# MarkJhonBao/InfantPoseEstimation_GaussianBias

Hardware: AMD Instinct MI355X
Metric: images/sec (train fwd+bwd) HRFormer-S 256x192 (higher is better)
Workload: dtype bf16; 1 GPU; HRFormer-small + fusion head, 256x192 -> 64x48, K=17, train step fwd+bwd+AdamW, DropPath 0.1, BN train; global_batch=64, per_gpu_batch=64, parallelism=dp1, launch=hipGraph replay, branches on concurrent HIP streams

## Files before the change

### infantposeestimation_gaussianbias_amd/csrc/pk_bn_out1x1.hip

```cpp
#include <stdlib.h>

#include "pk_rowops.h"

#define BO_ROWS 128
#define BO_GRID 512
#define BO_MIN_ROWS 32768
#define BO_SMALL_ROWS 32768

struct BnOutArgs {
    const uint4* raw;
    const uint16_t* w;
    const uint16_t* g;
    const uint8_t* mask_in;
    uint8_t* mask_out;
    const float* v0;
    const float* v1;
    const float* gamma;
    const float* sums;
    const float* bias;
    float* out;
    uint4* t_out;
    uint4* draw;
    float* part;
    float inv_count;
    int small;
    int64_t rows;
    int N, N8, hw, softplus;
    int nb, rpb;
};

template <int C>
struct BoGeom {
    static constexpr int CPR = C / 8;
    static constexpr int RPI = 64 / CPR;
    static constexpr int NLD = 16 / RPI;
    static constexpr int TP = C + 8;
    static constexpr int RL = 256 / CPR;
    static constexpr int TILE_BYTES = (16 * TP * 2 > RL * C * 4) ? 16 * TP * 2 : RL * C * 4;
};

__device__ __forceinline__ void bo_wave_sync() {
    __builtin_amdgcn_fence(__ATOMIC_ACQ_REL, "wavefront");
    __builtin_amdgcn_wave_barrier();
}

template <int C, int NB>
__global__ void __launch_bounds__(256, 2) k_bn_out1x1_fwd(BnOutArgs p) {
    using G = BoGeom<C>;
    constexpr int CPR = G::CPR, RPI = G::RPI, NLD = G::NLD, TP = G::TP;
    extern __shared__ __attribute__((aligned(16))) unsigned char bo_smem[];
    uint16_t* sW = reinterpret_cast<uint16_t*>(bo_smem);
    const int tid = threadIdx.x, lane = tid & 63, wave = tid >> 6;
    uint16_t* tile = reinterpret_cast<uint16_t*>(bo_smem + NB * 16 * TP * 2) + wave * 16 * TP;
    const int frow = lane & 15, fkc = lane >> 4;
    const int lch = lane % CPR, lrw = lane / CPR;
    const int64_t rows = p.rows;
    const int ntiles = (int)((rows + BO_ROWS - 1) / BO_ROWS);
    auto block_base = [&](int it) -> int64_t {
        const int64_t t = (int64_t)blockIdx.x + (int64_t)(it >> 1) * gridDim.x;
        return t < ntiles ? t * BO_ROWS + wave * 32 + (it & 1) * 16 : -1;
    };
    auto load_raw = [&](uint4 (&rv)[NLD], int64_t base) {
#pragma unroll
        for (int i = 0; i < NLD; ++i) {
            const int64_t row = base + i * RPI + lrw;
            rv[i] = make_uint4(0u, 0u, 0u, 0u);
            if (base >= 0 && row < rows) rv[i] = p.raw[(size_t)row * CPR + lch];
        }
    };
    uint4 rv[NLD], rn[NLD];
    int64_t base = block_base(0);
// ... 43 lines not shown
#pragma unroll
        for (int a = 0; a < NB; ++a) acc[a] = (f32x4){0.f, 0.f, 0.f, 0.f};
#pragma unroll
        for (int ks = 0; ks < C / 32; ++ks) {
            const bf16x8 tf = *reinterpret_cast<const bf16x8*>(&tile[frow * TP + (ks * 4 + fkc) * 8]);
#pragma unroll
            for (int a = 0; a < NB; ++a) {
                const bf16x8 wf = *reinterpret_cast<const bf16x8*>(&sW[(a * 16 + frow) * TP + (ks * 4 + fkc) * 8]);
                acc[a] = __builtin_amdgcn_mfma_f32_16x16x32_bf16(wf, tf, acc[a], 0, 0, 0);
            }
        }
        const int64_t row = base + frow;
        if (row < rows) {
            const int bb = (int)(row / p.hw), pix = (int)(row - (int64_t)bb * p.hw);
            float* o = p.out + (size_t)bb * p.N * p.hw + pix;
#pragma unroll
            for (int a = 0; a < NB; ++a)
#pragma unroll
                for (int r = 0; r < 4; ++r) {
                    const int n = a * 16 + fkc * 4 + r;
                    if (n < p.N) {
                        float v = acc[a][r] + bs[a][r];
                        if (p.softplus) v = softplus_(v);
                        o[(size_t)n * p.hw] = v;
                    }
                }
        }
#pragma unroll
        for (int i = 0; i < NLD; ++i) rv[i] = rn[i];
        base = nbase;
    }
}

template <int MODE, int C, int KP>
__global__ void __launch_bounds__(256, MODE == 1 ? 1 : 2) k_bn_out1x1_bwd(BnOutArgs p) {
    using G = BoGeom<C>;
    constexpr int CPR = G::CPR, RPI = G::RPI, NLD = G::NLD, TP = G::TP, RL = G::RL;
    constexpr int WP = KP + 8, KS = KP / 32;
    extern __shared__ __attribute__((aligned(16))) unsigned char bo_smem[];
    uint16_t* sWd = reinterpret_cast<uint16_t*>(bo_smem);
    float* sVec = reinterpret_cast<float*>(bo_smem + C * WP * 2);
    unsigned char* tiles = bo_smem + C * WP * 2 + 5 * C * 4;
    const int tid = threadIdx.x, lane = tid & 63, wave = tid >> 6;
    uint16_t* tile = reinterpret_cast<uint16_t*>(tiles + wave * G::TILE_BYTES);
    const int frow = lane & 15, fkc = lane >> 4;
    const int lch = lane % CPR, lrw = lane / CPR;
    const int64_t rows = p.rows;
    const int ntiles = (int)((rows + BO_ROWS - 1) / BO_ROWS);
    const int bpu = (p.rpb + 15) / 16;
    const int total_it = MODE == 1 ? ((p.nb + 4 * (int)gridDim.x - 1) / (4 * (int)gridDim.x)) * bpu : 0;
    auto position = [&](int it, int& unit, int64_t& base, int64_t& end) {
        base = end = 0;
        unit = -1;
        if (MODE == 1) {
            const int q = it / bpu, k = it - q * bpu;
            const int u = ((int)blockIdx.x + q * (int)gridDim.x) * 4 + wave;
            if (it < total_it && u < p.nb) {
                unit = u;
                base = (int64_t)u * p.rpb + 16 * k;
                end = min(rows, (int64_t)(u + 1) * p.rpb);
            }
        } else {
            const int64_t t = (int64_t)blockIdx.x + (int64_t)(it >> 1) * gridDim.x;
            if (t < ntiles) {
                unit = 0;
                base = t * BO_ROWS + wave * 32 + (it & 1) * 16;
                end = rows;
            }
        }
    };
    struct Block {
        uint4 rv[NLD];
        uint32_t mv[NLD];
        bf16x8 gf[KS];
    };
    auto load_block = [&](Block& b, int64_t base, int64_t end) {
#pragma unroll
        for (int i = 0; i < NLD; ++i) {
            const int64_t row = base + i * RPI + lrw;
            b.rv[i] = make_uint4(0u, 0u, 0u, 0u);
            b.mv[i] = 0u;
            if (row < end) {
                b.rv[i] = p.raw[(size_t)row * CPR + lch];
                b.mv[i] = p.mask_in[(size_t)row * CPR + lch];
            }
        }
#pragma unroll
        for (int ks = 0; ks < KS; ++ks) {
            const int64_t row = base + frow;
            b.gf[ks] = (bf16x8){0, 0, 0, 0, 0, 0, 0, 0};
            if (row < end && (ks * 4 + fkc) * 8 < p.N8) b.gf[ks] = *reinterpret_cast<const bf16x8*>(p.g + (size_t)row * p.N8 + (ks * 4 + fkc) * 8);
        }
    };
    Block cur, nxt, nx2;
    int unit, nunit;
    int64_t base, end, nbase, nend;
    position(0, unit, base, end);
    load_block(cur, base, end);
    position(1, nunit, nbase, nend);
    if (MODE == 1) load_block(nxt, nbase, nend);
    {
        const int wch = p.N8 / 8;
        for (int i = tid; i < C * (KP / 8); i += 256) {
            const int c = i / (KP / 8), ch = i - c * (KP / 8);
            u32x4 v = {0u, 0u, 0u, 0u};
            if (ch < wch) v = reinterpret_cast<const u32x4*>(p.w)[(size_t)c * wch + ch];
            *reinterpret_cast<u32x4*>(&sWd[c * WP + ch * 8]) = v;
        }
        for (int c = tid; c < C; c += 256) {
            sVec[c] = p.v0[c];
            sVec[C + c] = p.v1[c];
            if (MODE == 2) {
                sVec[2 * C + c] = p.gamma[c];
                sVec[3 * C + c] = p.sums[c];
                sVec[4 * C + c] = p.sums[C + c];
            }
        }
    }
    float s1[4][8], s2[4][8];
    if (MODE == 1) {
#pragma unroll
        for (int s = 0; s < 4; ++s)
#pragma unroll
            for (int j = 0; j < 8; ++j) s1[s][j] = s2[s][j] = 0.f;
    }
    __syncthreads();
    for (int it = 0; MODE == 1 ? it < total_it : unit >= 0; ++it) {
        int n2unit = -1;
        int64_t n2base = 0, n2end = 0;
        if (MODE == 1) {
            position(it + 2, n2unit, n2base, n2end);
            load_block(nx2, n2base, n2end);
        } else {
            load_block(nxt, nbase, nend);
        }
        bo_wave_sync();
#pragma unroll
        for (int cg = 0; cg < C / 64; ++cg) {
            f32x4 acc[4];
#pragma unroll
            for (int a = 0; a < 4; ++a) acc[a] = (f32x4){0.f, 0.f, 0.f, 0.f};
#pragma unroll
            for (int ks = 0; ks < KS; ++ks)
#pragma unroll
                for (int a = 0; a < 4; ++a) {
                    const bf16x8 wf = *reinterpret_cast<const bf16x8*>(&sWd[(cg * 64 + a * 16 + frow) * WP + (ks * 4 + fkc) * 8]);
                    acc[a] = __builtin_amdgcn_mfma_f32_16x16x32_bf16(wf, cur.gf[ks], acc[a], 0, 0, 0);
                }
#pragma unroll
            for (int a = 0; a < 4; ++a) {
                const u32x2 d = {pack_bf16x2(acc[a][0] + 0.f, acc[a][1] + 0.f), pack_bf16x2(acc[a][2] + 0.f, acc[a][3] + 0.f)};
                *reinterpret_cast<u32x2*>(&tile[frow * TP + cg * 64 + a * 16 + fkc * 4]) = d;
            }
        }
        bo_wave_sync();
        {
            float mu[8], rs[8], va[8], vb[8], vc[8];
            {
                const int c0 = lch * 8;
#pragma unroll
                for (int j = 0; j < 8; ++j) {
                    mu[j] = sVec[c0 + j];
                    rs[j] = sVec[C + c0 + j];
                    va[j] = MODE == 2 ? sVec[2 * C + c0 + j] : 0.f;
                    vb[j] = MODE == 2 ? sVec[3 * C + c0 + j] : 0.f;
                    vc[j] = MODE == 2 ? sVec[4 * C + c0 + j] : 0.f;
                }
            }
#pragma unroll
            for (int i = 0; i < NLD; ++i) {
                const int rl = i * RPI + lrw;
                const int64_t row = base + rl;
                const uint16_t* cell = &tile[rl * TP + lch * 8];
                if (row >= end) continue;
                float g[8], xr[8];
                unpack8(*reinterpret_cast<const uint4*>(cell), g);
                unpack8(cur.rv[i], xr);
                const uint32_t mb = cur.mv[i];
                if (MODE == 1) {
#pragma unroll
                    for (int j = 0; j < 8; ++j) {
                        const float gg = ((mb >> j) & 1u) ? g[j] : 0.f;
                        s1[i & 3][j] += gg;
                        s2[i & 3][j] += gg * (xr[j] - mu[j]) * rs[j];
                    }
                } else {
                    float o[8];
                    if (p.small) {
#pragma unroll
                        for (int j = 0; j < 8; ++j) {
                            const float gg = ((mb >> j) & 1u) ? g[j] : 0.f;
                            const float gm = va[j] * rs[j], t1 = vb[j] * p.inv_count, t2 = vc[j] * p.inv_count;
                            const float xh = (xr[j] - mu[j]) * rs[j];
                            o[j] = gm * (gg - t1 - xh * t2);
                        }
                    } else {
#pragma unroll
                        for (int j = 0; j < 8; ++j) {
                            const float gg = ((mb >> j) & 1u) ? g[j] : 0.f;
                            const float xh = (xr[j] - mu[j]) * rs[j];
                            o[j] = va[j] * rs[j] * (gg - vb[j] * p.inv_count - xh * vc[j] * p.inv_count);
                        }
                    }
                    p.draw[(size_t)row * CPR + lch] = pack8(o);
                }
            }
        }
        if (MODE == 1) {
            if (unit >= 0 && it - (it / bpu) * bpu == bpu - 1) {
                float* stage = reinterpret_cast<float*>(tile);
                float* dst = p.part + (size_t)unit * 2 * C;
#pragma unroll
                for (int h = 0; h < 2; ++h) {
                    bo_wave_sync();
#pragma unroll
                    for (int s = 0; s < 4; ++s)
#pragma unroll
                        for (int j = 0; j < 8; ++j) {
                            stage[(s * RPI + lrw) * C + lch * 8 + j] = h ? s2[s][j] : s1[s][j];
                            if (h) s1[s][j] = s2[s][j] = 0.f;
                        }
                    bo_wave_sync();
#pragma unroll
                    for (int q = 0; q < C / 64; ++q) {
                        float a = 0.f;
#pragma unroll
                        for (int k = 0; k < RL; ++k) a += stage[k * C + q * 64 + lane];
                        dst[h * C + q * 64 + lane] = a;
                    }
                }
                bo_wave_sync();
            }
        }
        cur = nxt;
        unit = nunit;
        base = nbase;
        end = nend;
        if (MODE == 1) {
            nxt = nx2;
            nunit = n2unit;
            nbase = n2base;
            nend = n2end;
        } else {
            position(it + 2, nunit, nbase, nend);
        }
    }
}

__global__ void __launch_bounds__(256) k_bn_out1x1_sum_small(const float* __restrict__ part, int nb, int C, float* __restrict__ sums,
                                                             float* __restrict__ dbeta, float* __restrict__ dgamma) {
    __shared__ double sh1[8][32], sh2[8][32];
    const int c0 = (int)blockIdx.x * 32;
    const int cl = threadIdx.x & 31, pl = threadIdx.x >> 5, c = c0 + cl;
    double a = 0.0, b = 0.0;
    if (c < C)
        for (int t = pl; t < nb; t += 8) {
            a += (double)part[(size_t)t * 2 * C + c];
            b += (double)part[(size_t)t * 2 * C + C + c];
        }
    sh1[pl][cl] = a;
    sh2[pl][cl] = b;
    __syncthreads();
    if (threadIdx.x < 32 && c < C) {
        a = b = 0.0;
#pragma unroll
        for (int k = 0; k < 8; ++k) {
            a += sh1[k][cl];
            b += sh2[k][cl];
        }
        sums[c] = (float)a;
        sums[C + c] = (float)b;
        dbeta[c] = (float)a;
        dgamma[c] = (float)b;
    }
}

static inline int bo_grid(int64_t want) {
    const char* cap = getenv("PK_BN_OUT1X1_MAX_GRID");
    int64_t lim = BO_GRID;
    if (cap && atoi(cap) >= 1 && atoi(cap) < BO_GRID) lim = atoi(cap);
    if (want > lim) want = lim;
    return (int)(want < 1 ? 1 : want);
}
static inline bool bo_shape_ok(int64_t rows, int C, int N) { return rows > 0 && rows < (1 << 30) && (C == 256 || C == 128) && N >= 1 && N <= 48; }
extern "C" int pk_bn_out1x1_supported(int64_t rows, int C, int N) {
    const char *on = getenv("PK_BN_OUT1X1"), *mr = getenv("PK_BN_OUT1X1_MIN_ROWS");
    if (on && on[0] == '0') return 0;
    int64_t min_rows = BO_MIN_ROWS;
    if (mr && atoll(mr) >= 1) min_rows = atoll(mr);
    return (bo_shape_ok(rows, C, N) && rows >= min_rows) ? 1 : 0;
}
static inline bool bo_aligned(const void* a, const void* b = nullptr, const void* c = nullptr, const void* d = nullptr) {
    return (((uintptr_t)a | (uintptr_t)b | (uintptr_t)c | (uintptr_t)d) & 15) == 0;
}
#define BO_CHECK_SHAPE(who)                                                     \
    PK_REQUIRE(rows > 0 && rows < (1 << 30) && N > 0, who ": bad sizes");       \
    PK_SUPPORTED(bo_shape_ok(rows, C, N), who ": built for C = 128 / 256 channels and N <= 48 outputs (got %d -> %d)", C, N)

static int bo_launch(void (*kernel)(BnOutArgs), bool& attr_set, int grid, int lds, const BnOutArgs& a, hipStream_t st, const char* who) {
    const hipError_t e = attr_set ? hipSuccess : hipFuncSetAttribute((const void*)kernel, hipFuncAttributeMaxDynamicSharedMemorySize, lds);
    if (e != hipSuccess) return pk_set_error("%s: cannot reserve %d bytes of LDS: %s", who, lds, hipGetErrorString(e)), (int)e;
    attr_set = true;
    hipLaunchKernelGGL(kernel, dim3((unsigned)grid), dim3(256), lds, st, a);
    return pk_launch_status(who);
}
template <int C, int NB>
static int bo_fwd(const BnOutArgs& a, hipStream_t st, const char* who) {
    static bool attr_set = false;
    const int lds = NB * 16 * BoGeom<C>::TP * 2 + 4 * 16 * BoGeom<C>::TP * 2;
    return bo_launch(k_bn_out1x1_fwd<C, NB>, attr_set, bo_grid((a.rows + BO_ROWS - 1) / BO_ROWS), lds, a, st, who);
}
template <int MODE, int C, int KP>
static int bo_bwd(const BnOutArgs& a, hipStream_t st, const char* who) {
    const int lds = C * (KP + 8) * 2 + 5 * C * 4 + 4 * BoGeom<C>::TILE_BYTES;
    const int grid = MODE == 1 ? bo_grid((a.nb + 3) / 4) : bo_grid((a.rows + BO_ROWS - 1) / BO_ROWS);
    static bool attr_set = false;
    return bo_launch(k_bn_out1x1_bwd<MODE, C, KP>, attr_set, grid, lds, a, st, who);
}
template <int MODE>
static int bo_bwd_any(const BnOutArgs& a, int C, hipStream_t st, const char* who) {
    if (C == 256) return a.N <= 32 ? bo_bwd<MODE, 256, 32>(a, st, who) : bo_bwd<MODE, 256, 64>(a, st, who);
    return a.N <= 32 ? bo_bwd<MODE, 128, 32>(a, st, who) : bo_bwd<MODE, 128, 64>(a, st, who);
}

extern "C" int pk_bn_out1x1_fwd(const void* raw, const float* scale, const float* shift, const void* w_fwd, const float* bias, void* t, float* out,
                                uint8_t* relu_mask, int64_t rows, int C, int N, int hw, int softplus, void* stream) {
    PK_REQUIRE(raw && scale && shift && w_fwd && bias && t && out && relu_mask, "pk_bn_out1x1_fwd: null pointer");
    BO_CHECK_SHAPE("pk_bn_out1x1_fwd");
    PK_REQUIRE(hw > 0 && rows % hw == 0, "pk_bn_out1x1_fwd: rows = %lld is no multiple of the plane size %d", (long long)rows, hw);
    PK_REQUIRE(bo_aligned(raw, w_fwd, t), "pk_bn_out1x1_fwd: raw, t and the weight must be 16-byte aligned");
    BnOutArgs a{};
    a.raw = (const uint4*)raw;
    a.w = (const uint16_t*)w_fwd;
    a.v0 = scale;
    a.v1 = shift;
    a.bias = bias;
    a.out = out;
    a.t_out = (uint4*)t;
    a.mask_out = relu_mask;
    a.rows = rows;
    a.N = N;
    a.hw = hw;
    a.softplus = softplus ? 1 : 0;
    hipStream_t st = (hipStream_t)stream;
    const char* who = "pk_bn_out1x1_fwd";
    if (C == 256) return N <= 32 ? bo_fwd<256, 2>(a, st, who) : bo_fwd<256, 3>(a, st, who);
    return N <= 32 ? bo_fwd<128, 2>(a, st, who) : bo_fwd<128, 3>(a, st, who);
}
// ... 34 lines not shown
```

### infantposeestimation_gaussianbias_amd/csrc/pk_conv1x1_bn.hip

```cpp
#include <stdlib.h>

#include "pk_rowops.h"

#define CB_ROWS 128
#define CB_CIN 64
#define CB_COUT 256
#define CB_EP 68
#define CB_W_BYTES (CB_COUT * CB_CIN * 2)
#define CB_STAGE_BYTES (4 * 32 * CB_EP * 4)
#define CB_VEC_BYTES (5 * CB_COUT * 4)
#define CB_LDS (CB_W_BYTES + CB_STAGE_BYTES + CB_VEC_BYTES)
#define CB_GRID 512
#define CB_MIN_ROWS 32768

struct Conv1x1Args {
    const uint16_t* x;
    const uint16_t* w;
    const uint4* in;
    const uint8_t* mask_in;
    const float* v0;
    const float* v1;
    const float* gamma;
    const float* sums;
    uint4* out;
    uint4* out2;
    uint8_t* mask_out;
    float* part;
    float inv_count;
    int64_t rows;
    int relu;
    int nb, rpb;
};

template <int MODE>
__global__ void __launch_bounds__(256, 2) k_conv1x1_bn(Conv1x1Args p) {
    extern __shared__ __attribute__((aligned(16))) unsigned char cb_smem[];
    uint16_t* sW = reinterpret_cast<uint16_t*>(cb_smem);
    float* sStage = reinterpret_cast<float*>(cb_smem + CB_W_BYTES);
    float* sVec = reinterpret_cast<float*>(cb_smem + CB_W_BYTES + CB_STAGE_BYTES);
    const int tid = threadIdx.x, lane = tid & 63, wave = tid >> 6;
    const int frow = lane & 15, fkc = lane >> 4;
    const int64_t rows = p.rows;
    const int ntiles = (int)((rows + CB_ROWS - 1) / CB_ROWS);
    const int lr = lane >> 3, lc = (lane & 7) * 8;
    float* stage = sStage + wave * 32 * CB_EP;
    auto wave_sync = [] {
        __builtin_amdgcn_fence(__ATOMIC_ACQ_REL, "wavefront");
        __builtin_amdgcn_wave_barrier();
    };
    auto load_x = [&](bf16x8 (&xf)[2][2], int64_t base, int64_t end) {
#pragma unroll
        for (int b = 0; b < 2; ++b) {
            const int64_t row = base + b * 16 + frow;
#pragma unroll
            for (int ks = 0; ks < 2; ++ks) {
                bf16x8 v = {0, 0, 0, 0, 0, 0, 0, 0};
                if (row < end) v = *reinterpret_cast<const bf16x8*>(p.x + (size_t)row * CB_CIN + ks * 32 + fkc * 8);
                xf[ks][b] = v;
            }
        }
    };
    auto load_in = [&](uint4 (&iv)[4], uint32_t (&mv)[4], int64_t base, int64_t end, int cg) {
#pragma unroll
        for (int ps = 0; ps < 4; ++ps) {
            const int64_t row = base + ps * 8 + lr;
            const size_t idx = (size_t)row * (CB_COUT / 8) + cg * 8 + (lane & 7);
            iv[ps] = make_uint4(0u, 0u, 0u, 0u);
            mv[ps] = 0xffu;
            if (row < end) {
                if (MODE >= 2 || (MODE == 1 && p.in)) iv[ps] = p.in[idx];
                if (MODE >= 2 && p.relu) mv[ps] = p.mask_in[idx];
            }
        }
    };

    auto position = [&](int t, int u, int k, int64_t& base, int64_t& end) {
        if (MODE == 2) {
            base = end = 0;
            if (u < p.nb) {
                base = (int64_t)u * p.rpb + 32 * k;
                end = min(rows, (int64_t)(u + 1) * p.rpb);
            }
        } else {
            base = (int64_t)t * CB_ROWS + wave * 32;
            end = rows;
        }
    };
    float s1[4][8], s2[4][8];
    if (MODE == 2) {
#pragma unroll
        for (int cg = 0; cg < 4; ++cg)
#pragma unroll
            for (int j = 0; j < 8; ++j) s1[cg][j] = s2[cg][j] = 0.f;
    }

    bf16x8 xf[2][2], xn[2][2];
    uint4 iv[2][4];
    uint32_t mv[2][4];
    int tile = (int)blockIdx.x, sbuf = 0;
    int unit = (int)blockIdx.x * 4 + wave, chunk = 0;
    int64_t base, end;
    position(tile, unit, chunk, base, end);
    load_x(xf, base, end);
    if (MODE >= 1) load_in(iv[0], mv[0], base, end, 0);
    for (int i = tid; i < CB_COUT * (CB_CIN / 8); i += 256) {
        const int row = i >> 3, ch = i & 7;
        *reinterpret_cast<u32x4*>(&sW[row * CB_CIN + ((ch ^ ((row >> 1) & 7)) * 8)]) = reinterpret_cast<const u32x4*>(p.w)[i];
    }
    if (MODE >= 1) {
        sVec[tid] = p.v0[tid];
        sVec[CB_COUT + tid] = p.v1[tid];
    }
    if (MODE == 3) {
        sVec[2 * CB_COUT + tid] = p.gamma[tid];
        sVec[3 * CB_COUT + tid] = p.sums[tid];
        sVec[4 * CB_COUT + tid] = p.sums[CB_COUT + tid];
    }
    __syncthreads();
    while (MODE == 2 ? unit < p.nb : tile < ntiles) {
        const bool unit_done = MODE == 2 && base + 32 >= end;
        const int tile_next = tile + (int)gridDim.x;
        const int unit_next = unit_done ? unit + (int)gridDim.x * 4 : unit, chunk_next = unit_done ? 0 : chunk + 1;
        int64_t nbase, nend;
        position(tile_next, unit_next, chunk_next, nbase, nend);
        load_x(xn, nbase, nend);
#pragma unroll
        for (int cg = 0; cg < 4; ++cg) {
            if (MODE >= 1) {
                if (cg < 3) load_in(iv[(cg + 1) & 1], mv[(cg + 1) & 1], base, end, cg + 1);
                else load_in(iv[0], mv[0], nbase, nend, 0);
            }
            f32x4 acc[4][2];
#pragma unroll
            for (int a = 0; a < 4; ++a)
#pragma unroll
                for (int b = 0; b < 2; ++b) acc[a][b] = (f32x4){0.f, 0.f, 0.f, 0.f};
#pragma unroll
            for (int ks = 0; ks < 2; ++ks) {
                bf16x8 wf[4];
#pragma unroll
                for (int a = 0; a < 4; ++a) {
                    const int n = cg * 64 + a * 16 + frow;
                    wf[a] = *reinterpret_cast<const bf16x8*>(&sW[n * CB_CIN + (((fkc + 4 * ks) ^ ((n >> 1) & 7)) * 8)]);
                }
#pragma unroll
                for (int a = 0; a < 4; ++a)
#pragma unroll
                    for (int b = 0; b < 2; ++b) acc[a][b] = __builtin_amdgcn_mfma_f32_16x16x32_bf16(wf[a], xf[ks][b], acc[a][b], 0, 0, 0);
            }
            if (MODE == 0) {
                float* sStat = sStage + sbuf * (4 * CB_COUT * 2);
#pragma unroll
                for (int a = 0; a < 4; ++a) {
#pragma unroll
                    for (int r = 0; r < 4; ++r) {
                        float s = 0.f, q = 0.f;
#pragma unroll
// ... 34 lines not shown
#pragma unroll
            for (int ps = 0; ps < 4; ++ps) {
                const int ml = ps * 8 + lr;
                const int64_t row = base + ml;
                if (row >= end) continue;
                const size_t idx = (size_t)row * (CB_COUT / 8) + cg * 8 + (lane & 7);
                const f32x4 lo = *reinterpret_cast<const f32x4*>(&stage[ml * CB_EP + lc]);
                const f32x4 hi = *reinterpret_cast<const f32x4*>(&stage[ml * CB_EP + lc + 4]);
                const float accv[8] = {lo[0], lo[1], lo[2], lo[3], hi[0], hi[1], hi[2], hi[3]};
                float xr[8];
                unpack8(pack8(accv), xr);
                const uint4 in = iv[cg & 1][ps];
                if (MODE == 1) {
                    float v[8];
#pragma unroll
                    for (int j = 0; j < 8; ++j) v[j] = xr[j] * va[j] + vb[j];
                    if (p.in) {
                        float r[8];
                        unpack8(in, r);
#pragma unroll
                        for (int j = 0; j < 8; ++j) v[j] += r[j];
                    }
                    if (p.relu) {
#pragma unroll
                        for (int j = 0; j < 8; ++j) v[j] = fmaxf(v[j], 0.f);
                    }
                    const uint4 o = pack8(v);
                    p.out[idx] = o;
                    if (p.mask_out) p.mask_out[idx] = (uint8_t)pos_mask8(o);
                } else {
                    float g[8];
                    unpack8(in, g);
                    const uint32_t mb = mv[cg & 1][ps];
                    if (MODE == 2) {
#pragma unroll
                        for (int j = 0; j < 8; ++j) {
                            const float gg = ((mb >> j) & 1u) ? g[j] : 0.f;
                            s1[cg][j] += gg;
                            s2[cg][j] += gg * (xr[j] - va[j]) * vb[j];
                        }
                    } else {
                        float o[8];
#pragma unroll
                        for (int j = 0; j < 8; ++j) {
                            const float gg = ((mb >> j) & 1u) ? g[j] : 0.f;
                            g[j] = gg;
                            const float xh = (xr[j] - va[j]) * vb[j];
                            o[j] = vc[j] * vb[j] * (gg - vd[j] * p.inv_count - xh * ve[j] * p.inv_count);
                        }
                        p.out[idx] = pack8(o);
                        if (p.out2) p.out2[idx] = pack8(g);
                    }
                }
            }
        }
        if (MODE == 0) {
            __syncthreads();
            const float* sStat = sStage + sbuf * (4 * CB_COUT * 2);
            float s = 0.f, q = 0.f;
#pragma unroll
            for (int w = 0; w < 4; ++w) {
                s += sStat[(w * CB_COUT + tid) * 2];
                q += sStat[(w * CB_COUT + tid) * 2 + 1];
            }
            float* dst = p.part + (size_t)tile * 2 * CB_COUT;
            dst[tid] = s;
            dst[CB_COUT + tid] = q;
            sbuf ^= 1;
        }
        if (MODE == 2 && unit_done) {
            float* dst = p.part + (size_t)unit * 2 * CB_COUT;
#pragma unroll
            for (int cg = 0; cg < 4; ++cg) {
                wave_sync();
#pragma unroll
                for (int j = 0; j < 8; ++j) {
                    stage[(lr * 2) * 64 + lc + j] = s1[cg][j];
                    stage[(lr * 2 + 1) * 64 + lc + j] = s2[cg][j];
                    s1[cg][j] = s2[cg][j] = 0.f;
                }
                wave_sync();
                float a = 0.f, b = 0.f;
#pragma unroll
                for (int k = 0; k < 8; ++k) {
                    a += stage[(k * 2) * 64 + lane];
                    b += stage[(k * 2 + 1) * 64 + lane];
                }
                dst[cg * 64 + lane] = a;
                dst[CB_COUT + cg * 64 + lane] = b;
            }
        }
#pragma unroll
        for (int ks = 0; ks < 2; ++ks)
#pragma unroll
            for (int b = 0; b < 2; ++b) xf[ks][b] = xn[ks][b];
        tile = tile_next;
        unit = unit_next;
        chunk = chunk_next;
        base = nbase;
        end = nend;
    }
}

static inline int cb_grid(int64_t rows) {
    const char* cap = getenv("PK_CONV1X1_BN_MAX_GRID");
    int64_t g = (rows + CB_ROWS - 1) / CB_ROWS;
    int64_t lim = CB_GRID;
    if (cap && atoi(cap) >= 1 && atoi(cap) < CB_GRID) lim = atoi(cap);
    if (g > lim) g = lim;
    return (int)(g < 1 ? 1 : g);
}
extern "C" int pk_conv1x1_bn_supported(int64_t rows, int Cin, int Cout) {
    const char *on = getenv("PK_CONV1X1_BN"), *mr = getenv("PK_CONV1X1_BN_MIN_ROWS");
    if (on && on[0] == '0') return 0;
    int64_t min_rows = CB_MIN_ROWS;
    if (mr && atoll(mr) >= 1) min_rows = atoll(mr);
    return (Cin == CB_CIN && Cout == CB_COUT && rows >= min_rows && rows < (1 << 30)) ? 1 : 0;
}
extern "C" int pk_conv1x1_stats_rows(int64_t rows) { return rows > 0 && rows < (1 << 30) ? (int)((rows + CB_ROWS - 1) / CB_ROWS) : 0; }
extern "C" int pk_conv1x1_bn_bwd_rows(int64_t rows) { return rows > 0 && rows < (1 << 30) ? pk_bn_bwd_blocks(rows) : 0; }

static inline bool cb_aligned(const void* a, const void* b = nullptr, const void* c = nullptr, const void* d = nullptr) {
    return (((uintptr_t)a | (uintptr_t)b | (uintptr_t)c | (uintptr_t)d) & 15) == 0;
}
#define CB_CHECK_SHAPE(who)                                                                                                       \
    PK_REQUIRE(rows > 0 && rows < (1 << 30), who ": bad row count");                                                             \
    PK_SUPPORTED(Cin == CB_CIN && Cout == CB_COUT, who ": built for Cin = 64, Cout = 256 (got %d -> %d)", Cin, Cout)

template <int MODE>
static int cb_launch(const Conv1x1Args& a, hipStream_t st, const char* who) {
    static bool attr_set = false;
    const hipError_t e = attr_set ? hipSuccess : hipFuncSetAttribute((const void*)k_conv1x1_bn<MODE>, hipFuncAttributeMaxDynamicSharedMemorySize, CB_LDS);
    if (e != hipSuccess) return pk_set_error("%s: cannot reserve %d bytes of LDS: %s", who, CB_LDS, hipGetErrorString(e)), (int)e;
    attr_set = true;
    const int grid = MODE == 2 ? cb_grid((int64_t)a.nb * 32) : cb_grid(a.rows);
    hipLaunchKernelGGL(k_conv1x1_bn<MODE>, dim3((unsigned)grid), dim3(256), CB_LDS, st, a);
    return pk_launch_status(who);
}

extern "C" int pk_conv1x1_stats(const void* x, const void* w, float* stats_partial, int64_t rows, int Cin, int Cout, void* stream) {
    PK_REQUIRE(x && w && stats_partial, "pk_conv1x1_stats: null pointer");
    CB_CHECK_SHAPE("pk_conv1x1_stats");
    PK_REQUIRE(cb_aligned(x, w), "pk_conv1x1_stats: x and w must be 16-byte aligned");
    Conv1x1Args a{};
    a.x = (const uint16_t*)x;
    a.w = (const uint16_t*)w;
    a.part = stats_partial;
    a.rows = rows;
    return cb_launch<0>(a, (hipStream_t)stream, "pk_conv1x1_stats");
}

extern "C" int pk_conv1x1_bn_act(const void* x, const void* w, const float* scale, const float* shift, const void* residual, void* y, int relu,
                                 uint8_t* relu_mask, int64_t rows, int Cin, int Cout, void* stream) {
    PK_REQUIRE(x && w && scale && shift && y, "pk_conv1x1_bn_act: null pointer");
    CB_CHECK_SHAPE("pk_conv1x1_bn_act");
    PK_REQUIRE(cb_aligned(x, w, residual, y), "pk_conv1x1_bn_act: tensors must be 16-byte aligned");
    Conv1x1Args a{};
    a.x = (const uint16_t*)x;
    a.w = (const uint16_t*)w;
    a.v0 = scale;
    a.v1 = shift;
    a.in = (const uint4*)residual;
    a.out = (uint4*)y;
    a.mask_out = relu_mask;
    a.relu = relu ? 1 : 0;
    a.rows = rows;
    return cb_launch<1>(a, (hipStream_t)stream, "pk_conv1x1_bn_act");
}

// ... 55 lines not shown
```

Baseline: 4323 images/sec.

## Split BN-backward reduction into a dedicated per-wave kernel body with smaller LDS

The MODE 1/2 statistics-reduction paths of the fused 1x1-conv BN backward kernels are split into standalone bodies. In these, each wave owns a 64-channel slice, keeps its weight fragments in a private LDS region, writes a swizzled 16x64 tile and triple-buffers its loads. LDS per block shrinks and launch bounds rise to 4 blocks per CU, with a larger grid cap, to raise occupancy and overlap memory with MFMA. The apply paths are simplified to drop the reduce-only branches. The trade-off is extra fixed per-wave setup, more partial-sum units and more complex indexing.

Measured after the change: 4343 images/sec (median of 6 runs). No clear change (+0.4%).

```diff
diff --git a/infantposeestimation_gaussianbias_amd/csrc/pk_bn_out1x1.hip b/infantposeestimation_gaussianbias_amd/csrc/pk_bn_out1x1.hip
--- a/infantposeestimation_gaussianbias_amd/csrc/pk_bn_out1x1.hip
+++ b/infantposeestimation_gaussianbias_amd/csrc/pk_bn_out1x1.hip
@@ -35,8 +35,7 @@
     static constexpr int RPI = 64 / CPR;
     static constexpr int NLD = 16 / RPI;
     static constexpr int TP = C + 8;
-    static constexpr int RL = 256 / CPR;
-    static constexpr int TILE_BYTES = (16 * TP * 2 > RL * C * 4) ? 16 * TP * 2 : RL * C * 4;
+    static constexpr int TILE_BYTES = 16 * TP * 2;
 };
 
 __device__ __forceinline__ void bo_wave_sync() {
@@ -146,10 +145,156 @@
     }
 }
 
-template <int MODE, int C, int KP>
-__global__ void __launch_bounds__(256, MODE == 1 ? 1 : 2) k_bn_out1x1_bwd(BnOutArgs p) {
+template <int C, int KP>
+struct BoRed {
+    static constexpr int CPR = C / 8;
+    static constexpr int RL = 256 / CPR;
+    static constexpr int NS = RL / 8;
+    static constexpr int WPU = C / 64, UPW = 4 / WPU;
+    static constexpr int KS = KP / 32;
+    static constexpr int W_BYTES = KS * 4 * 64 * 16;
+    static constexpr int TILE_BYTES = RL * 64 * 4 > 2048 ? RL * 64 * 4 : 2048;
+    static constexpr int WAVE_BYTES = W_BYTES + TILE_BYTES;
+};
+
+template <int C, int KP>
+__device__ __forceinline__ void bo_reduce_body(const BnOutArgs& p) {
+    using R = BoRed<C, KP>;
+    constexpr int CPR = R::CPR, RL = R::RL, NS = R::NS, WPU = R::WPU, UPW = R::UPW, KS = R::KS;
+    extern __shared__ __attribute__((aligned(16))) unsigned char bo_smem[];
+    const int lane = threadIdx.x & 63, wave = __builtin_amdgcn_readfirstlane(threadIdx.x >> 6);
+    const int cw = wave % WPU, usub = wave / WPU;
+    bf16x8* sWf = reinterpret_cast<bf16x8*>(bo_smem + wave * R::WAVE_BYTES);
+    uint16_t* tile = reinterpret_cast<uint16_t*>(bo_smem + wave * R::WAVE_BYTES + R::W_BYTES);
+    const int frow = lane & 15, fkc = lane >> 4;
+    const int lch = lane & 7, lrw = lane >> 3;
+    const int64_t rows = p.rows;
+    const int bpu = (p.rpb + 15) / 16;
+    const int rounds = (p.nb + UPW * (int)gridDim.x - 1) / (UPW * (int)gridDim.x);
+    struct Block {
+        uint4 rv[2];
+        uint32_t mv[2];
+        bf16x8 gf[KS];
+        int unit, n;
+        bool last;
+    };
+    int fq = 0, fk = 0;
+    auto fetch = [&](Block& b) {
+        const int u = ((int)blockIdx.x + fq * (int)gridDim.x) * UPW + usub;
+        const int64_t base = (int64_t)u * p.rpb + 16 * fk;
+        b.unit = u;
+        b.n = u < p.nb ? (int)min((int64_t)16, min(rows, (int64_t)(u + 1) * p.rpb) - base) : 0;
+        b.last = u < p.nb && fk == bpu - 1;
+        if (++fk == bpu) {
+            fk = 0;
+            ++fq;
+        }
+        const int64_t vb = b.n > 0 ? base : 0;
+        const size_t cb = (size_t)vb * CPR + cw * 8;
+        const uint16_t* gb = p.g + (size_t)vb * p.N8;
+#pragma unroll
+        for (int i = 0; i < 2; ++i) {
+            const int r = i * 8 + lrw < b.n ? i * 8 + lrw : 0;
+            const int idx = r * CPR + lch;
+            b.rv[i] = (p.raw + cb)[idx];
+            b.mv[i] = (p.mask_in + cb)[idx];
+        }
+        const int gr = frow < b.n ? frow : 0;
+#pragma unroll
+        for (int ks = 0; ks < KS; ++ks) {
+            const bool in = (ks * 4 + fkc) * 8 < p.N8;
+            const bf16x8 v = *reinterpret_cast<const bf16x8*>(gb + gr * p.N8 + (in ? (ks * 4 + fkc) * 8 : 0));
+            b.gf[ks] = in ? v : (bf16x8){0, 0, 0, 0, 0, 0, 0, 0};
+        }
+    };
+    Block b0, b1, b2;
+    fetch(b0);
+    fetch(b1);
+    {
+        const int wch = p.N8 / 8;
+#pragma unroll
+        for (int f = 0; f < KS * 4; ++f) {
+            const int c = cw * 64 + (f & 3) * 16 + frow, ch = (f >> 2) * 4 + fkc;
+            u32x4 v = {0u, 0u, 0u, 0u};
+            if (ch < wch) v = reinterpret_cast<const u32x4*>(p.w)[(size_t)c * wch + ch];
+            *reinterpret_cast<u32x4*>(&sWf[f * 64 + lane]) = v;
+        }
+    }
+    float mu[8], rs[8];
+#pragma unroll
+    for (int j = 0; j < 8; ++j) {
+        mu[j] = p.v0[cw * 64 + lch * 8 + j];
+        rs[j] = p.v1[cw * 64 + lch * 8 + j];
+    }
+    float s1[NS][8], s2[NS][8];
+#pragma unroll
+    for (int s = 0; s < NS; ++s)
+#pragma unroll
+        for (int j = 0; j < 8; ++j) s1[s][j] = s2[s][j] = 0.f;
+    auto step = [&](Block& cur, Block& spare) {
+        bo_wave_sync();
+        f32x4 acc[4];
+#pragma unroll
+        for (int a = 0; a < 4; ++a) acc[a] = (f32x4){0.f, 0.f, 0.f, 0.f};
+#pragma unroll
+        for (int ks = 0; ks < KS; ++ks)
+#pragma unroll
+            for (int a = 0; a < 4; ++a) acc[a] = __builtin_amdgcn_mfma_f32_16x16x32_bf16(sWf[(ks * 4 + a) * 64 + lane], cur.gf[ks], acc[a], 0, 0, 0);
+#pragma unroll
+        for (int a = 0; a < 4; ++a) {
+            const u32x2 d = {pack_bf16x2(acc[a][0] + 0.f, acc[a][1] + 0.f), pack_bf16x2(acc[a][2] + 0.f, acc[a][3] + 0.f)};
+            const int chunk = a * 2 + (fkc >> 1);
+            *reinterpret_cast<u32x2*>(&tile[frow * 64 + ((chunk ^ ((frow >> 1) & 7)) * 8) + (fkc & 1) * 4]) = d;
+        }
+        fetch(spare);
+        bo_wave_sync();
+#pragma unroll
+        for (int i = 0; i < 2; ++i) {
+            const int rl = i * 8 + lrw;
+            if (rl >= cur.n) continue;
+            float g[8], xr[8];
+            unpack8(*reinterpret_cast<const uint4*>(&tile[rl * 64 + ((lch ^ ((rl >> 1) & 7)) * 8)]), g);
+            unpack8(cur.rv[i], xr);
+            const uint32_t mb = cur.mv[i];
+#pragma unroll
+            for (int j = 0; j < 8; ++j) {
+                const float gg = ((mb >> j) & 1u) ? g[j] : 0.f;
+                s1[i % NS][j] += gg;
+                s2[i % NS][j] += gg * (xr[j] - mu[j]) * rs[j];
+            }
+        }
+        if (cur.last) {
+            float* stage = reinterpret_cast<float*>(tile);
+            float* dst = p.part + (size_t)cur.unit * 2 * C + cw * 64;
+#pragma unroll
+            for (int h = 0; h < 2; ++h) {
+                bo_wave_sync();
+#pragma unroll
+                for (int s = 0; s < NS; ++s)
+#pragma unroll
+                    for (int j = 0; j < 8; ++j) {
+                        stage[(s * 8 + lrw) * 64 + lch * 8 + j] = h ? s2[s][j] : s1[s][j];
+                        if (h) s1[s][j] = s2[s][j] = 0.f;
+                    }
+                bo_wave_sync();
+                float a = 0.f;
+#pragma unroll
+                for (int k = 0; k < RL; ++k) a += stage[k * 64 + lane];
+                dst[h * C + lane] = a;
+            }
+        }
+    };
+    for (int it = 0; it < rounds * bpu; it += 3) {
+        step(b0, b2);
+        step(b1, b0);
+        step(b2, b1);
+    }
+}
+
+template <int C, int KP>
+__device__ __forceinline__ void bo_apply_body(const BnOutArgs& p) {
     using G = BoGeom<C>;
-    constexpr int CPR = G::CPR, RPI = G::RPI, NLD = G::NLD, TP = G::TP, RL = G::RL;
+    constexpr int CPR = G::CPR, RPI = G::RPI, NLD = G::NLD, TP = G::TP;
     constexpr int WP = KP + 8, KS = KP / 32;
     extern __shared__ __attribute__((aligned(16))) unsigned char bo_smem[];
     uint16_t* sWd = reinterpret_cast<uint16_t*>(bo_smem);
@@ -161,26 +306,14 @@
     const int lch = lane % CPR, lrw = lane / CPR;
     const int64_t rows = p.rows;
     const int ntiles = (int)((rows + BO_ROWS - 1) / BO_ROWS);
-    const int bpu = (p.rpb + 15) / 16;
-    const int total_it = MODE == 1 ? ((p.nb + 4 * (int)gridDim.x - 1) / (4 * (int)gridDim.x)) * bpu : 0;
     auto position = [&](int it, int& unit, int64_t& base, int64_t& end) {
         base = end = 0;
         unit = -1;
-        if (MODE == 1) {
-            const int q = it / bpu, k = it - q * bpu;
-            const int u = ((int)blockIdx.x + q * (int)gridDim.x) * 4 + wave;
-            if (it < total_it && u < p.nb) {
-                unit = u;
-                base = (int64_t)u * p.rpb + 16 * k;
-                end = min(rows, (int64_t)(u + 1) * p.rpb);
-            }
-        } else {
-            const int64_t t = (int64_t)blockIdx.x + (int64_t)(it >> 1) * gridDim.x;
-            if (t < ntiles) {
-                unit = 0;
-                base = t * BO_ROWS + wave * 32 + (it & 1) * 16;
-                end = rows;
-            }
+        const int64_t t = (int64_t)blockIdx.x + (int64_t)(it >> 1) * gridDim.x;
+        if (t < ntiles) {
+            unit = 0;
+            base = t * BO_ROWS + wave * 32 + (it & 1) * 16;
+            end = rows;
         }
     };
     struct Block {
@@ -206,13 +339,12 @@
             if (row < end && (ks * 4 + fkc) * 8 < p.N8) b.gf[ks] = *reinterpret_cast<const bf16x8*>(p.g + (size_t)row * p.N8 + (ks * 4 + fkc) * 8);
         }
     };
-    Block cur, nxt, nx2;
+    Block cur, nxt;
     int unit, nunit;
     int64_t base, end, nbase, nend;
     position(0, unit, base, end);
     load_block(cur, base, end);
     position(1, nunit, nbase, nend);
-    if (MODE == 1) load_block(nxt, nbase, nend);
     {
         const int wch = p.N8 / 8;
         for (int i = tid; i < C * (KP / 8); i += 256) {
@@ -224,30 +356,14 @@
         for (int c = tid; c < C; c += 256) {
             sVec[c] = p.v0[c];
             sVec[C + c] = p.v1[c];
-            if (MODE == 2) {
-                sVec[2 * C + c] = p.gamma[c];
-                sVec[3 * C + c] = p.sums[c];
-                sVec[4 * C + c] = p.sums[C + c];
-            }
-        }
-    }
-    float s1[4][8], s2[4][8];
-    if (MODE == 1) {
-#pragma unroll
-        for (int s = 0; s < 4; ++s)
-#pragma unroll
-            for (int j = 0; j < 8; ++j) s1[s][j] = s2[s][j] = 0.f;
+            sVec[2 * C + c] = p.gamma[c];
+            sVec[3 * C + c] = p.sums[c];
+            sVec[4 * C + c] = p.sums[C + c];
+        }
     }
     __syncthreads();
-    for (int it = 0; MODE == 1 ? it < total_it : unit >= 0; ++it) {
-        int n2unit = -1;
-        int64_t n2base = 0, n2end = 0;
-        if (MODE == 1) {
-            position(it + 2, n2unit, n2base, n2end);
-            load_block(nx2, n2base, n2end);
-        } else {
-            load_block(nxt, nbase, nend);
-        }
+    for (int it = 0; unit >= 0; ++it) {
+        load_block(nxt, nbase, nend);
         bo_wave_sync();
 #pragma unroll
         for (int cg = 0; cg < C / 64; ++cg) {
@@ -276,9 +392,9 @@
                 for (int j = 0; j < 8; ++j) {
                     mu[j] = sVec[c0 + j];
                     rs[j] = sVec[C + c0 + j];
-                    va[j] = MODE == 2 ? sVec[2 * C + c0 + j] : 0.f;
-                    vb[j] = MODE == 2 ? sVec[3 * C + c0 + j] : 0.f;
-                    vc[j] = MODE == 2 ? sVec[4 * C + c0 + j] : 0.f;
+                    va[j] = sVec[2 * C + c0 + j];
+                    vb[j] = sVec[3 * C + c0 + j];
+                    vc[j] = sVec[4 * C + c0 + j];
                 }
             }
 #pragma unroll
@@ -291,74 +407,38 @@
                 unpack8(*reinterpret_cast<const uint4*>(cell), g);
                 unpack8(cur.rv[i], xr);
                 const uint32_t mb = cur.mv[i];
-                if (MODE == 1) {
+                float o[8];
+                if (p.small) {
 #pragma unroll
                     for (int j = 0; j < 8; ++j) {
                         const float gg = ((mb >> j) & 1u) ? g[j] : 0.f;
-                        s1[i & 3][j] += gg;
-                        s2[i & 3][j] += gg * (xr[j] - mu[j]) * rs[j];
+                        const float gm = va[j] * rs[j], t1 = vb[j] * p.inv_count, t2 = vc[j] * p.inv_count;
+                        const float xh = (xr[j] - mu[j]) * rs[j];
+                        o[j] = gm * (gg - t1 - xh * t2);
                     }
                 } else {
-                    float o[8];
-                    if (p.small) {
-#pragma unroll
-                        for (int j = 0; j < 8; ++j) {
-                            const float gg = ((mb >> j) & 1u) ? g[j] : 0.f;
-                            const float gm = va[j] * rs[j], t1 = vb[j] * p.inv_count, t2 = vc[j] * p.inv_count;
-                            const float xh = (xr[j] - mu[j]) * rs[j];
-                            o[j] = gm * (gg - t1 - xh * t2);
-                        }
-                    } else {
-#pragma unroll
-                        for (int j = 0; j < 8; ++j) {
-                            const float gg = ((mb >> j) & 1u) ? g[j] : 0.f;
-                            const float xh = (xr[j] - mu[j]) * rs[j];
-                            o[j] = va[j] * rs[j] * (gg - vb[j] * p.inv_count - xh * vc[j] * p.inv_count);
-                        }
-                    }
-                    p.draw[(size_t)row * CPR + lch] = pack8(o);
-                }
-            }
-        }
-        if (MODE == 1) {
-            if (unit >= 0 && it - (it / bpu) * bpu == bpu - 1) {
-                float* stage = reinterpret_cast<float*>(tile);
-                float* dst = p.part + (size_t)unit * 2 * C;
-#pragma unroll
-                for (int h = 0; h < 2; ++h) {
-                    bo_wave_sync();
-#pragma unroll
-                    for (int s = 0; s < 4; ++s)
-#pragma unroll
-                        for (int j = 0; j < 8; ++j) {
-                            stage[(s * RPI + lrw) * C + lch * 8 + j] = h ? s2[s][j] : s1[s][j];
-                            if (h) s1[s][j] = s2[s][j] = 0.f;
-                        }
-                    bo_wave_sync();
-#pragma unroll
-                    for (int q = 0; q < C / 64; ++q) {
-                        float a = 0.f;
-#pragma unroll
-                        for (int k = 0; k < RL; ++k) a += stage[k * C + q * 64 + lane];
-                        dst[h * C + q * 64 + lane] = a;
+#pragma unroll
+                    for (int j = 0; j < 8; ++j) {
+                        const float gg = ((mb >> j) & 1u) ? g[j] : 0.f;
+                        const float xh = (xr[j] - mu[j]) * rs[j];
+                        o[j] = va[j] * rs[j] * (gg - vb[j] * p.inv_count - xh * vc[j] * p.inv_count);
                     }
                 }
-                bo_wave_sync();
+                p.draw[(size_t)row * CPR + lch] = pack8(o);
             }
         }
         cur = nxt;
         unit = nunit;
         base = nbase;
         end = nend;
-        if (MODE == 1) {
-            nxt = nx2;
-            nunit = n2unit;
-            nbase = n2base;
-            nend = n2end;
-        } else {
-            position(it + 2, nunit, nbase, nend);
-        }
-    }
+        position(it + 2, nunit, nbase, nend);
+    }
+}
+
+template <int MODE, int C, int KP>
+__global__ void __launch_bounds__(256, MODE == 2 || C == 128 ? 2 : 4) k_bn_out1x1_bwd(BnOutArgs p) {
+    if constexpr (MODE == 1) bo_reduce_body<C, KP>(p);
+    else bo_apply_body<C, KP>(p);
 }
 
 __global__ void __launch_bounds__(256) k_bn_out1x1_sum_small(const float* __restrict__ part, int nb, int C, float* __restrict__ sums,
@@ -389,10 +469,9 @@
     }
 }
 
-static inline int bo_grid(int64_t want) {
+static inline int bo_grid(int64_t want, int64_t lim = BO_GRID) {
     const char* cap = getenv("PK_BN_OUT1X1_MAX_GRID");
-    int64_t lim = BO_GRID;
-    if (cap && atoi(cap) >= 1 && atoi(cap) < BO_GRID) lim = atoi(cap);
+    if (cap && atoi(cap) >= 1 && atoi(cap) < lim) lim = atoi(cap);
     if (want > lim) want = lim;
     return (int)(want < 1 ? 1 : want);
 }
@@ -426,8 +505,9 @@
 }
 template <int MODE, int C, int KP>
 static int bo_bwd(const BnOutArgs& a, hipStream_t st, const char* who) {
-    const int lds = C * (KP + 8) * 2 + 5 * C * 4 + 4 * BoGeom<C>::TILE_BYTES;
-    const int grid = MODE == 1 ? bo_grid((a.nb + 3) / 4) : bo_grid((a.rows + BO_ROWS - 1) / BO_ROWS);
+    using R = BoRed<C, KP>;
+    const int lds = MODE == 1 ? 4 * R::WAVE_BYTES : C * (KP + 8) * 2 + 5 * C * 4 + 4 * BoGeom<C>::TILE_BYTES;
+    const int grid = MODE == 1 ? bo_grid((a.nb + R::UPW - 1) / R::UPW, 2 * BO_GRID) : bo_grid((a.rows + BO_ROWS - 1) / BO_ROWS);
     static bool attr_set = false;
     return bo_launch(k_bn_out1x1_bwd<MODE, C, KP>, attr_set, grid, lds, a, st, who);
 }
diff --git a/infantposeestimation_gaussianbias_amd/csrc/pk_conv1x1_bn.hip b/infantposeestimation_gaussianbias_amd/csrc/pk_conv1x1_bn.hip
--- a/infantposeestimation_gaussianbias_amd/csrc/pk_conv1x1_bn.hip
+++ b/infantposeestimation_gaussianbias_amd/csrc/pk_conv1x1_bn.hip
@@ -32,8 +32,135 @@
     int nb, rpb;
 };
 
+__device__ __forceinline__ void cb_wave_sync() {
+    __builtin_amdgcn_fence(__ATOMIC_ACQ_REL, "wavefront");
+    __builtin_amdgcn_wave_barrier();
+}
+
+#define CBR_W_BYTES (2 * 4 * 64 * 16)
+#define CBR_TILE_BYTES 2048
+#define CBR_LDS (4 * (CBR_W_BYTES + CBR_TILE_BYTES))
+#define CBR_GRID 1024
+__device__ __forceinline__ void cb_reduce_body(const Conv1x1Args& p) {
+    extern __shared__ __attribute__((aligned(16))) unsigned char cb_smem[];
+    const int lane = threadIdx.x & 63, cw = __builtin_amdgcn_readfirstlane(threadIdx.x >> 6);
+    bf16x8* sWf = reinterpret_cast<bf16x8*>(cb_smem + cw * (CBR_W_BYTES + CBR_TILE_BYTES));
+    uint16_t* tile = reinterpret_cast<uint16_t*>(cb_smem + cw * (CBR_W_BYTES + CBR_TILE_BYTES) + CBR_W_BYTES);
+    const int frow = lane & 15, fkc = lane >> 4;
+    const int lch = lane & 7, lrw = lane >> 3;
+    const int64_t rows = p.rows;
+    const int bpu = (p.rpb + 15) / 16;
+    const int rounds = (p.nb + (int)gridDim.x - 1) / (int)gridDim.x;
+    struct Block {
+        bf16x8 xf[2];
+        uint4 iv[2];
+        uint32_t mv[2];
+        int unit, n;
+        bool last;
+    };
+    int fq = 0, fk = 0;
+    auto fetch = [&](Block& b) {
+        const int u = (int)blockIdx.x + fq * (int)gridDim.x;
+        const int64_t base = (int64_t)u * p.rpb + 16 * fk;
+        b.unit = u;
+        b.n = u < p.nb ? (int)min((int64_t)16, min(rows, (int64_t)(u + 1) * p.rpb) - base) : 0;
+        b.last = u < p.nb && fk == bpu - 1;
+        if (++fk == bpu) {
+            fk = 0;
+            ++fq;
+        }
+        const int64_t vb = b.n > 0 ? base : 0;
+        const uint16_t* xb = p.x + (size_t)vb * CB_CIN;
+        const size_t cb = (size_t)vb * (CB_COUT / 8) + cw * 8;
+        const uint8_t* mb = p.relu ? p.mask_in : reinterpret_cast<const uint8_t*>(p.in);
+        const int xr = frow < b.n ? frow : 0;
+#pragma unroll
+        for (int ks = 0; ks < 2; ++ks) b.xf[ks] = *reinterpret_cast<const bf16x8*>(xb + xr * CB_CIN + ks * 32 + fkc * 8);
+#pragma unroll
+        for (int i = 0; i < 2; ++i) {
+            const int r = i * 8 + lrw < b.n ? i * 8 + lrw : 0;
+            const int idx = r * (CB_COUT / 8) + lch;
+            b.iv[i] = (p.in + cb)[idx];
+            b.mv[i] = (mb + cb)[idx] | (p.relu ? 0u : 0xffu);
+        }
+    };
+    Block b0, b1, b2;
+    fetch(b0);
+    fetch(b1);
+#pragma unroll
+    for (int f = 0; f < 8; ++f) {
+        const int n = cw * 64 + (f & 3) * 16 + frow, ch = (f >> 2) * 4 + fkc;
+        *reinterpret_cast<u32x4*>(&sWf[f * 64 + lane]) = reinterpret_cast<const u32x4*>(p.w)[n * (CB_CIN / 8) + ch];
+    }
+    float mu[8], rs[8];
+#pragma unroll
+    for (int j = 0; j < 8; ++j) {
+        mu[j] = p.v0[cw * 64 + lch * 8 + j];
+        rs[j] = p.v1[cw * 64 + lch * 8 + j];
+    }
+    float s1[8], s2[8];
+#pragma unroll
+    for (int j = 0; j < 8; ++j) s1[j] = s2[j] = 0.f;
+    auto step = [&](Block& cur, Block& spare) {
+        cb_wave_sync();
+        f32x4 acc[4];
+#pragma unroll
+        for (int a = 0; a < 4; ++a) acc[a] = (f32x4){0.f, 0.f, 0.f, 0.f};
+#pragma unroll
+        for (int ks = 0; ks < 2; ++ks)
+#pragma unroll
+            for (int a = 0; a < 4; ++a) acc[a] = __builtin_amdgcn_mfma_f32_16x16x32_bf16(sWf[(ks * 4 + a) * 64 + lane], cur.xf[ks], acc[a], 0, 0, 0);
+#pragma unroll
+        for (int a = 0; a < 4; ++a) {
+            const u32x2 d = {pack_bf16x2(acc[a][0], acc[a][1]), pack_bf16x2(acc[a][2], acc[a][3])};
+            const int chunk = a * 2 + (fkc >> 1);
+            *reinterpret_cast<u32x2*>(&tile[frow * 64 + ((chunk ^ ((frow >> 1) & 7)) * 8) + (fkc & 1) * 4]) = d;
+        }
+        fetch(spare);
+        cb_wave_sync();
+#pragma unroll
+        for (int i = 0; i < 2; ++i) {
+            const int rl = i * 8 + lrw;
+            if (rl >= cur.n) continue;
+            float g[8], xr[8];
+            unpack8(*reinterpret_cast<const uint4*>(&tile[rl * 64 + ((lch ^ ((rl >> 1) & 7)) * 8)]), xr);
+            unpack8(cur.iv[i], g);
+            const uint32_t mb = cur.mv[i];
+#pragma unroll
+            for (int j = 0; j < 8; ++j) {
+                const float gg = ((mb >> j) & 1u) ? g[j] : 0.f;
+                s1[j] += gg;
+                s2[j] += gg * (xr[j] - mu[j]) * rs[j];
+            }
+        }
+        if (cur.last) {
+            float* stage = reinterpret_cast<float*>(tile);
+            float* dst = p.part + (size_t)cur.unit * 2 * CB_COUT + cw * 64;
+#pragma unroll
+            for (int h = 0; h < 2; ++h) {
+                cb_wave_sync();
+#pragma unroll
+                for (int j = 0; j < 8; ++j) {
+                    stage[lrw * 64 + lch * 8 + j] = h ? s2[j] : s1[j];
+                    if (h) s1[j] = s2[j] = 0.f;
+                }
+                cb_wave_sync();
+                float a = 0.f;
+#pragma unroll
+                for (int k = 0; k < 8; ++k) a += stage[k * 64 + lane];
+                dst[h * CB_COUT + lane] = a;
+            }
+        }
+    };
+    for (int it = 0; it < rounds * bpu; it += 3) {
+        step(b0, b2);
+        step(b1, b0);
+        step(b2, b1);
+    }
+}
+
 template <int MODE>
-__global__ void __launch_bounds__(256, 2) k_conv1x1_bn(Conv1x1Args p) {
+__device__ __forceinline__ void cb_panel_body(const Conv1x1Args& p) {
     extern __shared__ __attribute__((aligned(16))) unsigned char cb_smem[];
     uint16_t* sW = reinterpret_cast<uint16_t*>(cb_smem);
     float* sStage = reinterpret_cast<float*>(cb_smem + CB_W_BYTES);
@@ -44,10 +171,7 @@
     const int ntiles = (int)((rows + CB_ROWS - 1) / CB_ROWS);
     const int lr = lane >> 3, lc = (lane & 7) * 8;
     float* stage = sStage + wave * 32 * CB_EP;
-    auto wave_sync = [] {
-        __builtin_amdgcn_fence(__ATOMIC_ACQ_REL, "wavefront");
-        __builtin_amdgcn_wave_barrier();
-    };
+    auto wave_sync = [] { cb_wave_sync(); };
     auto load_x = [&](bf16x8 (&xf)[2][2], int64_t base, int64_t end) {
 #pragma unroll
         for (int b = 0; b < 2; ++b) {
@@ -68,39 +192,22 @@
             iv[ps] = make_uint4(0u, 0u, 0u, 0u);
             mv[ps] = 0xffu;
             if (row < end) {
-                if (MODE >= 2 || (MODE == 1 && p.in)) iv[ps] = p.in[idx];
-                if (MODE >= 2 && p.relu) mv[ps] = p.mask_in[idx];
-            }
-        }
-    };
-
-    auto position = [&](int t, int u, int k, int64_t& base, int64_t& end) {
-        if (MODE == 2) {
-            base = end = 0;
-            if (u < p.nb) {
-                base = (int64_t)u * p.rpb + 32 * k;
-                end = min(rows, (int64_t)(u + 1) * p.rpb);
-            }
-        } else {
-            base = (int64_t)t * CB_ROWS + wave * 32;
-            end = rows;
-        }
-    };
-    float s1[4][8], s2[4][8];
-    if (MODE == 2) {
-#pragma unroll
-        for (int cg = 0; cg < 4; ++cg)
-#pragma unroll
-            for (int j = 0; j < 8; ++j) s1[cg][j] = s2[cg][j] = 0.f;
-    }
+                if (MODE == 3 || (MODE == 1 && p.in)) iv[ps] = p.in[idx];
+                if (MODE == 3 && p.relu) mv[ps] = p.mask_in[idx];
+            }
+        }
+    };
+    auto position = [&](int t, int64_t& base, int64_t& end) {
+        base = (int64_t)t * CB_ROWS + wave * 32;
+        end = rows;
+    };
 
     bf16x8 xf[2][2], xn[2][2];
     uint4 iv[2][4];
     uint32_t mv[2][4];
     int tile = (int)blockIdx.x, sbuf = 0;
-    int unit = (int)blockIdx.x * 4 + wave, chunk = 0;
     int64_t base, end;
-    position(tile, unit, chunk, base, end);
+    position(tile, base, end);
     load_x(xf, base, end);
     if (MODE >= 1) load_in(iv[0], mv[0], base, end, 0);
     for (int i = tid; i < CB_COUT * (CB_CIN / 8); i += 256) {
@@ -117,12 +224,10 @@
         sVec[4 * CB_COUT + tid] = p.sums[CB_COUT + tid];
     }
     __syncthreads();
-    while (MODE == 2 ? unit < p.nb : tile < ntiles) {
-        const bool unit_done = MODE == 2 && base + 32 >= end;
+    while (tile < ntiles) {
         const int tile_next = tile + (int)gridDim.x;
-        const int unit_next = unit_done ? unit + (int)gridDim.x * 4 : unit, chunk_next = unit_done ? 0 : chunk + 1;
         int64_t nbase, nend;
-        position(tile_next, unit_next, chunk_next, nbase, nend);
+        position(tile_next, nbase, nend);
         load_x(xn, nbase, nend);
 #pragma unroll
         for (int cg = 0; cg < 4; ++cg) {
@@ -223,25 +328,16 @@
                     float g[8];
                     unpack8(in, g);
                     const uint32_t mb = mv[cg & 1][ps];
-                    if (MODE == 2) {
-#pragma unroll
-                        for (int j = 0; j < 8; ++j) {
-                            const float gg = ((mb >> j) & 1u) ? g[j] : 0.f;
-                            s1[cg][j] += gg;
-                            s2[cg][j] += gg * (xr[j] - va[j]) * vb[j];
-                        }
-                    } else {
-                        float o[8];
-#pragma unroll
-                        for (int j = 0; j < 8; ++j) {
-                            const float gg = ((mb >> j) & 1u) ? g[j] : 0.f;
-                            g[j] = gg;
-                            const float xh = (xr[j] - va[j]) * vb[j];
-                            o[j] = vc[j] * vb[j] * (gg - vd[j] * p.inv_count - xh * ve[j] * p.inv_count);
-                        }
-                        p.out[idx] = pack8(o);
-                        if (p.out2) p.out2[idx] = pack8(g);
+                    float o[8];
+#pragma unroll
+                    for (int j = 0; j < 8; ++j) {
+                        const float gg = ((mb >> j) & 1u) ? g[j] : 0.f;
+                        g[j] = gg;
+                        const float xh = (xr[j] - va[j]) * vb[j];
+                        o[j] = vc[j] * vb[j] * (gg - vd[j] * p.inv_count - xh * ve[j] * p.inv_count);
                     }
+                    p.out[idx] = pack8(o);
+                    if (p.out2) p.out2[idx] = pack8(g);
                 }
             }
         }
@@ -259,45 +355,25 @@
             dst[CB_COUT + tid] = q;
             sbuf ^= 1;
         }
-        if (MODE == 2 && unit_done) {
-            float* dst = p.part + (size_t)unit * 2 * CB_COUT;
-#pragma unroll
-            for (int cg = 0; cg < 4; ++cg) {
-                wave_sync();
-#pragma unroll
-                for (int j = 0; j < 8; ++j) {
-                    stage[(lr * 2) * 64 + lc + j] = s1[cg][j];
-                    stage[(lr * 2 + 1) * 64 + lc + j] = s2[cg][j];
-                    s1[cg][j] = s2[cg][j] = 0.f;
-                }
-                wave_sync();
-                float a = 0.f, b = 0.f;
-#pragma unroll
-                for (int k = 0; k < 8; ++k) {
-                    a += stage[(k * 2) * 64 + lane];
-                    b += stage[(k * 2 + 1) * 64 + lane];
-                }
-                dst[cg * 64 + lane] = a;
-                dst[CB_COUT + cg * 64 + lane] = b;
-            }
-        }
 #pragma unroll
         for (int ks = 0; ks < 2; ++ks)
 #pragma unroll
             for (int b = 0; b < 2; ++b) xf[ks][b] = xn[ks][b];
         tile = tile_next;
-        unit = unit_next;
-        chunk = chunk_next;
         base = nbase;
         end = nend;
     }
 }
 
-static inline int cb_grid(int64_t rows) {
+template <int MODE>
+__global__ void __launch_bounds__(256, MODE == 2 ? 4 : 2) k_conv1x1_bn(Conv1x1Args p) {
+    if constexpr (MODE == 2) cb_reduce_body(p);
+    else cb_panel_body<MODE>(p);
+}
+
+static inline int cb_grid(int64_t g, int64_t lim = CB_GRID) {
     const char* cap = getenv("PK_CONV1X1_BN_MAX_GRID");
-    int64_t g = (rows + CB_ROWS - 1) / CB_ROWS;
-    int64_t lim = CB_GRID;
-    if (cap && atoi(cap) >= 1 && atoi(cap) < CB_GRID) lim = atoi(cap);
+    if (cap && atoi(cap) >= 1 && atoi(cap) < lim) lim = atoi(cap);
     if (g > lim) g = lim;
     return (int)(g < 1 ? 1 : g);
 }
@@ -321,11 +397,12 @@
 template <int MODE>
 static int cb_launch(const Conv1x1Args& a, hipStream_t st, const char* who) {
     static bool attr_set = false;
-    const hipError_t e = attr_set ? hipSuccess : hipFuncSetAttribute((const void*)k_conv1x1_bn<MODE>, hipFuncAttributeMaxDynamicSharedMemorySize, CB_LDS);
-    if (e != hipSuccess) return pk_set_error("%s: cannot reserve %d bytes of LDS: %s", who, CB_LDS, hipGetErrorString(e)), (int)e;
+    constexpr int lds = MODE == 2 ? CBR_LDS : CB_LDS;
+    const hipError_t e = attr_set ? hipSuccess : hipFuncSetAttribute((const void*)k_conv1x1_bn<MODE>, hipFuncAttributeMaxDynamicSharedMemorySize, lds);
+    if (e != hipSuccess) return pk_set_error("%s: cannot reserve %d bytes of LDS: %s", who, lds, hipGetErrorString(e)), (int)e;
     attr_set = true;
-    const int grid = MODE == 2 ? cb_grid((int64_t)a.nb * 32) : cb_grid(a.rows);
-    hipLaunchKernelGGL(k_conv1x1_bn<MODE>, dim3((unsigned)grid), dim3(256), CB_LDS, st, a);
+    const int grid = MODE == 2 ? cb_grid(a.nb, CBR_GRID) : cb_grid((a.rows + CB_ROWS - 1) / CB_ROWS);
+    hipLaunchKernelGGL(k_conv1x1_bn<MODE>, dim3((unsigned)grid), dim3(256), lds, st, a);
     return pk_launch_status(who);
 }
 
```
